# marvinquiet/SpaDOT

Hardware: AMD Instinct MI355X
Metric: training steps/sec + Sinkhorn iters/sec, 50k spots x 3k genes x 5 timepoints (higher is better)
Workload: dtype bf16; 1 GPU; cfg3: 5 time points x 10000 spots x 3000 genes, batch 512, k=30, 1200 inducing points; parallelism=1 GPU, n_sub=9980, E_sub=308893, m_inducing=236, params=16136032, hip_graphs=True, staged_graphs=True, bucketed_grad_exchange=False, units_in_schedule=80

## Files before the change

### include/spadot_model.h

```cpp
#ifndef SPADOT_MODEL_H
#define SPADOT_MODEL_H

#ifdef __cplusplus
extern "C" {
#endif

enum { SPADOT_DT_F32 = 0, SPADOT_DT_BF16 = 1, SPADOT_DT_F64 = 2 };
enum { SPADOT_KERNEL_GAUSSIAN = 0, SPADOT_KERNEL_CAUCHY = 1, SPADOT_KERNEL_QUADRATIC = 2 };

const char *spadot_model_version(void);

int spadot_gat_forward(const void *h, int dtype, const float *s_src, const float *s_dst,
                       const int *rowptr, const int *col, const float *bias, int n, int H, int C,
                       int concat, int act, void *out, float *alpha_out, void *stream);

int spadot_gat_backward_target(const void *g_out, const void *out, const void *h, int dtype,
                               const float *s_src, const float *s_dst, const float *alpha,
                               const int *rowptr, const int *col, int n, int H, int C, int concat,
                               int act, void *g_pre, float *dz, float *ds_dst, void *stream);

int spadot_gat_backward_source(const void *g_pre, int dtype, const float *alpha, const float *dz,
                               const int *rowptr_t, const int *col_t, const int *eid_t, int n, int H,
                               int C, void *dh, float *ds_src, const float *ds_dst, const float *att_src,
                               const float *att_dst, void *stream);
// ... 92 lines not shown
int spadot_kmeans_assign(const void *x, const void *centers, int n, int k, int d, int dtype, int *labels,
                         void *stream);

int spadot_sgemm_small(int mode, const float *A, int lda, const float *B, int ldb, float *C, int ldc, int M, int N, int K,
                       const float *bias, int batch, long long strideA, long long strideB, long long strideC, void *stream);

int spadot_enc_fused_supported(int b, int F1, int F2, int Q);
long long spadot_enc_fused_workspace(int b, int F1, int F2, int Q);
int spadot_enc_bn_map(const float *h1, const float *lin_bias, const float *gamma, const float *beta, float *running_mean,
                      float *running_var, long long *num_batches_tracked, int b, int F1, double momentum, double eps, double slope,
                      float *y1, float *save_mean, float *save_invstd, const float *W2, int F2, float *part, void *stream);
int spadot_enc_bn_fc(const float *part, int nparts, const float *lin_bias, const float *gamma, const float *beta, float *running_mean,
                     float *running_var, long long *num_batches_tracked, int b, int F2, double momentum, double eps, double slope,
                     float *h2, float *y2, float *save_mean, float *save_invstd, const float *Wfc, int Q, float *pz, void *stream);
int spadot_enc_sum_z(const float *pz, int nparts, const float *bias, int b, int Q, float *z, void *stream);
int spadot_svgp_pre2_partials(const float *pz, int nparts, const float *bias, const double *Kn, int b, int L, int m, float *z,
                              double *mu, double *var, double *w, double *muw, double *A, void *stream);

int spadot_recon_fb_supported(int b, int K, int G);
long long spadot_recon_fb_workspace(int b, int K, int G);
int spadot_recon_fb(const void *h_bf16, const void *W_bf16, const void *WT_bf16, int ldt, const float *bias, const float *y, int b, int K,
                    int G, double inv_scale, const float *grad_weight, void *g_bf16, float *workspace, double *loss_parts, float *dh,
                    void *stream);
int spadot_sum_parts(const double *part, int n, double scale, float *out, void *stream);

int spadot_stamp(unsigned long long *buf, int slot, void *stream);

int spadot_lloyd_step(const double *X, double *C, const int *xoff, const int *npts, int n_max, int R, const int *rgroup,
                      const int *Kr, int K_max, int D, const double *tol, double *part, int *done, double *inertia, int skip_done,
                      void *stream);
int spadot_kmeanspp_seed(const double *X, const int *xoff, const int *npts, int D, int P, const int *pset, const int *pK,
                         const int *pfirst, const int *puoff, const double *U, int K_max, int n_max, double *closest, int *idx,
                         double *centers, void *stream);

int spadot_knn(const double *x, int n, int d, int kk, int *out, void *stream);

int spadot_gat_mfma_supported(int dtype, int H, int C, int max_cols);

int spadot_gat_tail_supported(int dtype, int H, int K);
int spadot_gat_tail_wvec(const float *W, int ldw, const float *att_src, const float *att_dst, int H, int C, int K, float *part,
                         int slices, float *wv, void *whi, void *wlo, void *stream);
int spadot_gat_tail_logits(const void *x, int dtype, int ldx, const float *wv, const void *whi, const void *wlo, int n, int H, int K,
                           float *s, void *stream);
int spadot_gat_tail_aggregate(const void *x, int dtype, int ldx, const float *s, const int *rowptr, const int *col, int n_tgt, int H,
                              int K, void *A, float *alpha, void *stream);
int spadot_gat_tail_headmean(const void *O, int dtype, const float *bias, int n_tgt, int H, int C, void *out, void *stream);
// ... 37 lines not shown
int spadot_gemm_wgrad_bf16(const void *G, int ldg, const void *X, int ldx, float *dW, int ldw, int M, int N, int K,
                           int slices, float *workspace, const void *zero_row, void *stream);
long long spadot_gemm_wgrad_bf16_workspace_tiled(int M, int N, int K, int slices, int tile_k);
int spadot_gemm_wgrad_bf16_tiled(const void *G, int ldg, const void *X, int ldx, float *dW, int ldw, int M, int N, int K,
                                 int slices, int tile_k, float *workspace, const void *zero_row, void *stream);

int spadot_mlp_chain_supported(int n_layers, const int *dims);
int spadot_mlp_chain_workspace(int b, int n_layers, const int *dims, int *n_rows, int *width);
int spadot_mlp_chain_forward(const float *x, int b, int n_layers, const int *dims, const float *const *W,
                             const float *const *bias, const float *const *gamma, const float *const *beta, const double *eps,
                             const double *slope, float *const *a, float *const *y, float *const *mean, float *const *invstd,
                             void *stream);
int spadot_mlp_chain_forward_bf16(const float *x, int b, int n_layers, const int *dims, const float *const *W,
                                  const float *const *bias, const float *const *gamma, const float *const *beta,
                                  const double *eps, const double *slope, float *const *a, float *const *y, float *const *mean,
                                  float *const *invstd, void *y_last_bf16, void *stream);
int spadot_mlp_chain_backward(const float *dy, const float *x, int b, int n_layers, const int *dims, const float *const *W,
                              const float *const *gamma, const double *slope, float *const *a, float *const *y,
                              float *const *mean, float *const *invstd, float *dx, float *workspace, float *grads, void *stream);
int spadot_mlp_chain_backward_add(const float *dy, const float *x, int b, int n_layers, const int *dims, const float *const *W,
                                  const float *const *gamma, const double *slope, float *const *a, float *const *y,
                                  float *const *mean, float *const *invstd, float *dx, const float *dx_add, float *workspace,
                                  float *grads, void *stream);

int spadot_bias_sqerr_forward(const float *o, const float *bias, const float *y, int b, int G, double inv_scale, double *scratch,
                              float *out, void *stream);
int spadot_bias_sqerr_backward(const float *g1, const float *o, const float *bias, const float *y, int b, int G,
                               double inv_scale, void *g_bf16, float *dbias, void *stream);

int spadot_headfc_backward(const float *g, const void *h_bf16, const float *W, int b, int K, int N, void *dh_bf16,
                           float *workspace , float *grads ,
                           void *stream);

int spadot_cast_rows_multi(const float *const *src, void *const *dst, const int *rows, const int *K, const int *Kp, int n,
                           void *stream);

int spadot_grad_sumsq(const float *grad, long long count, double *scratch, float *sumsq, void *stream);
int spadot_clip_adamw_dev(float *param, const float *grad, float *exp_avg, float *exp_avg_sq, long long count, double lr,
                          double beta1, double beta2, double eps, double weight_decay, double max_norm, double *scratch,
                          float *sumsq, int *step_dev, unsigned *counter, const float *grad_scale_dev, void *stream);
typedef struct spadot_weight_image {
    long long offset;
    int rows, K, Kp, reserved;
    void *image;
} spadot_weight_image;
typedef struct spadot_weight_images {
// ... 79 lines not shown
```

### spadot_amd/_lib.py

```python
import ctypes
import os

_CSRC = os.path.join(os.path.dirname(os.path.abspath(__file__)), "csrc")
_CACHE = {}


class NativeLibraryMissing(RuntimeError):
    pass


def _load(name):
    if name in _CACHE:
        return _CACHE[name]
    import torch

    path = os.path.join(_CSRC, name)
    if not os.path.exists(path):
        raise NativeLibraryMissing(
            f"{path} is missing: build the HIP extension with `python -m spadot_amd.csrc.build` "
            "(needs hipcc; cross-compiles for gfx950 without a GPU). There is no CPU fallback.")
    lib = ctypes.CDLL(path)
    _CACHE[name] = lib
    return lib

# ... 148 lines not shown
        "spadot_gemm_tn_bf16": [vp, ci, vp, ci, vp, ci, ci, ci, ci, vp],
        "spadot_gemm_nn_bf16": [vp, ci, vp, ci, vp, ci, ci, ci, ci, vp],
        "spadot_enc_fused_supported": [ci, ci, ci, ci],
        "spadot_recon_fb_supported": [ci, ci, ci],
        "spadot_recon_fb": [vp, vp, vp, ci, vp, vp, ci, ci, ci, cd, vp, vp, vp, vp, vp, vp],
        "spadot_sum_parts": [vp, ci, cd, vp, vp],
        "spadot_enc_bn_map": [vp, vp, vp, vp, vp, vp, vp, ci, ci, cd, cd, cd, vp, vp, vp, vp, ci, vp, vp],
        "spadot_enc_bn_fc": [vp, ci, vp, vp, vp, vp, vp, vp, ci, ci, cd, cd, cd, vp, vp, vp, vp, vp, ci, vp, vp],
        "spadot_enc_sum_z": [vp, ci, vp, ci, ci, vp, vp],
        "spadot_svgp_pre2_partials": [vp, ci, vp, vp, ci, ci, ci, vp, vp, vp, vp, vp, vp, vp],
        "spadot_gemm_nn_bf16_masked": [vp, ci, vp, ci, vp, ci, ci, ci, ci, vp, ci, cd, vp],
        "spadot_gemm_tn_bf16_split": [vp, ci, vp, ci, vp, ci, ci, ci, ci, ci, ci, vp, vp],
        "spadot_gemm_wgrad_bf16": [vp, ci, vp, ci, vp, ci, ci, ci, ci, ci, vp, vp, vp],
        "spadot_gemm_wgrad_bf16_tiled": [vp, ci, vp, ci, vp, ci, ci, ci, ci, ci, ci, vp, vp, vp],
        "spadot_mlp_chain_supported": [ci, vp],
        "spadot_headfc_backward": [vp, vp, vp, ci, ci, ci, vp, vp, vp, vp],
        "spadot_bias_sqerr_forward": [vp, vp, vp, ci, ci, cd, vp, vp, vp],
        "spadot_bias_sqerr_backward": [vp, vp, vp, vp, ci, ci, cd, vp, vp, vp],
        "spadot_mlp_chain_workspace": [ci, ci, vp, vp, vp],
        "spadot_mlp_chain_forward": [vp, ci, ci, vp, vp, vp, vp, vp, vp, vp, vp, vp, vp, vp, vp],
        "spadot_mlp_chain_forward_bf16": [vp, ci, ci, vp, vp, vp, vp, vp, vp, vp, vp, vp, vp, vp, vp, vp],
        "spadot_mlp_chain_backward": [vp, vp, ci, ci, vp, vp, vp, vp, vp, vp, vp, vp, vp, vp, vp, vp],
        "spadot_mlp_chain_backward_add": [vp, vp, ci, ci, vp, vp, vp, vp, vp, vp, vp, vp, vp, vp, vp, vp, vp],
        "spadot_kernel_matrix": [vp, vp, ci, ci, ci, cd, ci, ci, vp, vp],
        "spadot_spd_inverse_logdet": [vp, ci, ci, vp, vp, vp],
        "spadot_rowdot_forward": [vp, vp, ci, ci, ci, ci, vp, vp],
        "spadot_rowdot_backward": [vp, vp, ci, ci, ci, ci, vp, vp],
        "spadot_elbo_forward": [vp, vp, vp, vp, vp, vp, vp, ci, ci, ci, vp, vp],
        "spadot_elbo_backward": [vp, vp, vp, vp, vp, vp, vp, vp, ci, ci, ci, vp, vp, vp, vp, vp, vp, vp],
        "spadot_bn_act_forward": [vp, ci, vp, vp, vp, vp, vp, vp, ci, ci, cd, cd, cd, vp, vp, vp, vp],
        "spadot_bn_act_backward": [vp, vp, vp, ci, vp, vp, vp, vp, ci, ci, cd, vp, vp, vp, vp],
        "spadot_ln_act_forward": [vp, vp, vp, ci, ci, cd, cd, vp, vp, vp, vp],
        "spadot_ln_act_backward": [vp, vp, vp, vp, vp, vp, ci, ci, cd, vp, vp, vp, vp],
        "spadot_svgp_post_forward": [vp] * 9 + [ci, ci, ci, cd, cd, cd] + [vp] * 7,
        "spadot_svgp_post_backward": [vp] * 13 + [ci, ci, ci, cd, cd] + [vp] * 8,
        "spadot_svgp_grad_tail": [vp] * 11 + [ci, ci, cd] + [vp] * 4,
        "spadot_svgp_q1t": [vp, vp, vp, vp, vp, ci, ci, ci, vp, vp],
        "spadot_svgp_post_pm_pv": [vp, vp, vp, ci, ci, cd, vp, vp, vp],
        "spadot_svgp_pre": [vp, ci, ci, vp, vp, vp, vp, vp],
        "spadot_svgp_pre2": [vp, vp, ci, ci, ci, vp, vp, vp, vp, vp, vp],
        "spadot_svgp_mid": [vp, vp, vp, vp, ci, ci, ci, vp, vp, vp, vp, vp, ci, vp],
        "spadot_spd_inverse_logdet2": [vp, ci, ci, ci, vp, vp, vp, vp, vp],
        "spadot_latent_head_forward": [vp, vp, vp, vp, ci, ci, ci, vp, vp, vp, vp, vp, vp],
        "spadot_latent_head_backward": [vp, vp, vp, vp, vp, vp, vp, ci, ci, ci, vp, vp, vp, vp],
        "spadot_cluster_losses_forward": [vp, vp, vp, vp, vp, vp, vp, ci, ci, ci, ci, ci, ci, ci, vp, vp, vp],
        "spadot_cluster_losses_backward": [vp, vp, vp, vp, vp, vp, vp, vp, ci, ci, ci, ci, ci, ci, ci, vp, vp],
# ... 64 lines not shown
```

### spadot_amd/csrc/mlp_chain.hip

```cpp
#include <hip/hip_runtime.h>
#include <cstdint>

#include "../../include/spadot_model.h"
#include "per_device.h"

namespace {

constexpr int MAXL = 4, MAXD = 256, WAVE = 64;
constexpr int RBF = 4;
constexpr int RBB = 8;
constexpr int LDW = MAXD + 4;

typedef float f32x4 __attribute__((ext_vector_type(4)));

struct Stage {
    const float *W, *bias, *gamma, *beta;
    float *a, *y, *mean, *invstd;
    int din, dout;
    float eps, slope;
    int ws_off;
};
struct Chain {
    Stage s[MAXL];
    int n;
// ... 58 lines not shown
            float ss = 0.f;
            for (int j = lane; j < dout; j += WAVE) { const float d = ar[j] - mean; ss += d * d; }
            const float invstd = rsqrtf(wave_sum(ss) / (float)dout + s.eps);
            for (int j = lane; j < dout; j += WAVE) {
                const float av = ar[j];
                const float v = (av - mean) * invstd * par[1][j] + par[2][j];
                const float yv = v > 0.f ? v : s.slope * v;
                ar[j] = yv;
                if (row < b) {
                    s.a[(size_t)row * dout + j] = av; s.y[(size_t)row * dout + j] = yv;
                    if (ch.ybf && l == ch.n - 1) ch.ybf[(size_t)row * dout + j] = (__bf16)yv;
                }
            }
            if (lane == 0 && row < b) { s.mean[row] = mean; s.invstd[row] = invstd; }
        }
        __syncthreads();
        cur ^= 1;
    }
}

constexpr int WST = 16384;
constexpr int LPR = 256 / RBB;
constexpr int LDS_BWD_FLOATS = 4 * RBB * LDW + 2 * RBB + MAXD + WST;
__global__ __launch_bounds__(256, 1) void k_mlp_chain_bwd(const float *__restrict__ dy_last, const float *__restrict__ x, int b,
                                                       Chain ch, float *__restrict__ dx_out, float *__restrict__ ws,
                                                       int ws_width, const float *__restrict__ dx_add) {
    extern __shared__ __attribute__((aligned(16))) float lds_dyn[];
    float (*gz)[LDW] = reinterpret_cast<float (*)[LDW]>(lds_dyn);
    float (*da)[LDW] = reinterpret_cast<float (*)[LDW]>(lds_dyn + RBB * LDW);
    float (*xs)[LDW] = reinterpret_cast<float (*)[LDW]>(lds_dyn + 2 * RBB * LDW);
    float (*xh)[LDW] = reinterpret_cast<float (*)[LDW]>(lds_dyn + 3 * RBB * LDW);
    float *rmean = lds_dyn + 4 * RBB * LDW, *rinv = rmean + RBB;
    float *gam = rinv + RBB;
    float *wst = gam + MAXD;
    const int t = threadIdx.x;
    const int r0 = blockIdx.x * RBB;
    float *wrow = ws + (size_t)blockIdx.x * ws_width;
    {
        const int d = ch.s[ch.n - 1].dout;
        float v[RBB * MAXD / 256];
#pragma unroll
        for (int u = 0; u < RBB * MAXD / 256; u++) {
            const int e = min(t + u * 256, RBB * d - 1), r = e / d, j = e - r * d;
            v[u] = dy_last[(size_t)min(r0 + r, b - 1) * d + j];
        }
#pragma unroll
        for (int u = 0; u < RBB * MAXD / 256; u++) {
            const int e = t + u * 256;
            if (!(e < RBB * d && r0 + e / d < b)) v[u] = 0.f;
        }
#pragma unroll
        for (int u = 0; u < RBB * MAXD / 256; u++) {
            const int e = t + u * 256, r = e / d, j = e - r * d;
            if (e < RBB * d) gz[r][j] = v[u];
        }
    }
    for (int l = ch.n - 1; l >= 0; l--) {
        const Stage &s = ch.s[l];
        const int din = s.din, dout = s.dout;
        const float *xin = l == 0 ? x : ch.s[l - 1].y;
        const int tk = din / 4;
        const int jc = min(dout, WST / din);
        const bool need_dx = l > 0 || dx_out != nullptr;
        {
            constexpr int NE = RBB * MAXD / 256, NW = WST / 4 / 256;
            float vx[NE], vy[NE], va[NE];
            f32x4 vw[NW];
#pragma unroll
            for (int u = 0; u < NE; u++) {
                const int e = min(t + u * 256, RBB * din - 1), r = e / din, k = e - r * din;
                vx[u] = xin[(size_t)min(r0 + r, b - 1) * din + k];
                const int e2 = min(t + u * 256, RBB * dout - 1), r2 = e2 / dout, j = e2 - r2 * dout;
                const size_t o2 = (size_t)min(r0 + r2, b - 1) * dout + j;
                vy[u] = s.y[o2];
                va[u] = s.a[o2];
            }
            {
                const f32x4 *src = reinterpret_cast<const f32x4 *>(s.W);
#pragma unroll
                for (int u = 0; u < NW; u++) vw[u] = src[min(t + u * 256, jc * tk - 1)];
            }
            const int rr = min(r0 + (t & (RBB - 1)), b - 1);
            const float mean_t = s.mean[rr], inv_t = s.invstd[rr], gam_t = s.gamma[min(t, dout - 1)];
#pragma unroll
            for (int u = 0; u < NE; u++) {
                const int e = t + u * 256;
                if (!(e < RBB * din && r0 + e / din < b)) vx[u] = 0.f;
                if (!(e < RBB * dout && r0 + e / dout < b)) { vy[u] = 0.f; va[u] = 0.f; }
            }
            if (t < RBB) {
                const bool live = r0 + t < b;
                rmean[t] = live ? mean_t : 0.f;
                rinv[t] = live ? inv_t : 0.f;
            }
            if (t < dout) gam[t] = gam_t;
            __syncthreads();
#pragma unroll
            for (int u = 0; u < NE; u++) {
                const int e = t + u * 256;
                if (e < RBB * din) { const int r = e / din; xs[r][e - r * din] = vx[u]; }
                if (e < RBB * dout) {
                    const int r = e / dout, j = e - r * dout;
                    const bool live = r0 + r < b;
                    gz[r][j] = live ? gz[r][j] * (vy[u] > 0.f ? 1.f : s.slope) : 0.f;
                    xh[r][j] = live ? (va[u] - rmean[r]) * rinv[r] : 0.f;
                }
// ... 94 lines not shown
                            const float4 w = *reinterpret_cast<const float4 *>(wst + (size_t)j * din + k0);
                            a4.x += d * w.x; a4.y += d * w.y; a4.z += d * w.z; a4.w += d * w.w;
                        }
                        acc[u] = a4;
                    }
                }
            }
#pragma unroll
            for (int u = 0; u < 4; u++) {
                const int e = it0 + u * 128;
                if (half == 1 && e < nitem) *reinterpret_cast<float4 *>(&xh[0][0] + 4 * e) = acc[u];
            }
            __syncthreads();
#pragma unroll
            for (int u = 0; u < 4; u++) {
                const int e = it0 + u * 128;
                if (half == 0 && e < nitem) {
                    const int r = e / tk, k0 = (e - r * tk) * 4;
                    const float4 o = *reinterpret_cast<const float4 *>(&xh[0][0] + 4 * e);
                    const float4 a4 = make_float4(acc[u].x + o.x, acc[u].y + o.y, acc[u].z + o.z, acc[u].w + o.w);
                    if (l > 0) *reinterpret_cast<float4 *>(&gz[r][k0]) = a4;
                    else if (r0 + r < b) {
                        float4 o4 = a4;
                        if (dx_add) {
                            const float4 e4 = *reinterpret_cast<const float4 *>(dx_add + (size_t)(r0 + r) * din + k0);
                            o4 = make_float4(a4.x + e4.x, a4.y + e4.y, a4.z + e4.z, a4.w + e4.w);
                        }
                        *reinterpret_cast<float4 *>(dx_out + (size_t)(r0 + r) * din + k0) = o4;
                    }
                }
            }
        }
        __syncthreads();
    }
}

__device__ __forceinline__ double block_sum_d(double x, double *sh) {
#pragma unroll
    for (int off = 32; off > 0; off >>= 1) x += __shfl_xor(x, off, WAVE);
    const int w = threadIdx.x >> 6, nw = (blockDim.x + 63) >> 6;
    __syncthreads();
    if ((threadIdx.x & 63) == 0) sh[w] = x;
    __syncthreads();
    double t = 0.0;
    for (int k = 0; k < nw; k++) t += sh[k];
    return t;
}

constexpr int SQ_ROWS = 1;
__global__ __launch_bounds__(256) void k_bias_sqerr_part(const float *__restrict__ o, const float *__restrict__ bias,
                                                         const float *__restrict__ y, int b, int G,
                                                         double *__restrict__ part) {
    __shared__ double sh[16];
    const size_t row = (size_t)blockIdx.x * G;
    double acc = 0.0;
    for (int c0 = threadIdx.x; c0 < G; c0 += 4 * 256) {
// ... 160 lines not shown
    *n_rows = (b + RBB - 1) / RBB;
    *width = w;
    return 0;
}

int spadot_mlp_chain_forward_bf16(const float *x, int b, int n_layers, const int *dims, const float *const *W,
                                  const float *const *bias, const float *const *gamma, const float *const *beta,
                                  const double *eps, const double *slope, float *const *a, float *const *y, float *const *mean,
                                  float *const *invstd, void *y_last_bf16, void *stream) {
    Chain ch;
    if (b <= 0 || !fill_chain(ch, n_layers, dims, W, bias, gamma, beta, eps, slope, a, y, mean, invstd)) return -22;
    ch.ybf = (__bf16 *)y_last_bf16;
    hipLaunchKernelGGL(k_mlp_chain_fwd, dim3((b + RBF - 1) / RBF), dim3(256), 0, (hipStream_t)stream, x, b, ch);
    return hipGetLastError() == hipSuccess ? 0 : -5;
}

int spadot_mlp_chain_forward(const float *x, int b, int n_layers, const int *dims, const float *const *W,
                             const float *const *bias, const float *const *gamma, const float *const *beta, const double *eps,
                             const double *slope, float *const *a, float *const *y, float *const *mean, float *const *invstd,
                             void *stream) {
    return spadot_mlp_chain_forward_bf16(x, b, n_layers, dims, W, bias, gamma, beta, eps, slope, a, y, mean, invstd, nullptr, stream);
}

int spadot_mlp_chain_backward_add(const float *dy, const float *x, int b, int n_layers, const int *dims, const float *const *W,
                                  const float *const *gamma, const double *slope, float *const *a, float *const *y,
                                  float *const *mean, float *const *invstd, float *dx, const float *dx_add, float *workspace,
                                  float *grads, void *stream) {
    Chain ch;
    if (b <= 0 || !fill_chain(ch, n_layers, dims, W, nullptr, gamma, nullptr, nullptr, slope, a, y, mean, invstd)) return -22;
    if (dx_add && !dx) return -22;
    int rows, width;
    if (spadot_mlp_chain_workspace(b, n_layers, dims, &rows, &width)) return -22;
    constexpr int LDS_BWD = LDS_BWD_FLOATS * (int)sizeof(float);
    static PerDeviceFlag attr_set;     
    if (!attr_set) {
        if (hipFuncSetAttribute((const void *)k_mlp_chain_bwd, hipFuncAttributeMaxDynamicSharedMemorySize, LDS_BWD) != hipSuccess) return -5;
        attr_set = true;
    }
    hipLaunchKernelGGL(k_mlp_chain_bwd, dim3(rows), dim3(256), LDS_BWD, (hipStream_t)stream, dy, x, b, ch, dx, workspace, width, dx_add);
    if (hipGetLastError() != hipSuccess) return -5;
    if (!grads) return 0;
    return spadot_colsum(workspace, rows, width, grads, stream);
}

int spadot_mlp_chain_backward(const float *dy, const float *x, int b, int n_layers, const int *dims, const float *const *W,
                              const float *const *gamma, const double *slope, float *const *a, float *const *y,
                              float *const *mean, float *const *invstd, float *dx, float *workspace, float *grads, void *stream) {
    return spadot_mlp_chain_backward_add(dy, x, b, n_layers, dims, W, gamma, slope, a, y, mean, invstd, dx, nullptr, workspace, grads,
                                         stream);
}

int spadot_bias_sqerr_forward(const float *o, const float *bias, const float *y, int b, int G, double inv_scale, double *scratch,
                              float *out, void *stream) {
    const int nb = (b + SQ_ROWS - 1) / SQ_ROWS;
    if (b <= 0 || G <= 0 || !scratch || nb > 4096) return -22;
    hipLaunchKernelGGL(k_bias_sqerr_part, dim3(nb), dim3(256), 0, (hipStream_t)stream, o, bias, y, b, G, scratch);
    hipLaunchKernelGGL(k_sum_parts, dim3(1), dim3(1024), 0, (hipStream_t)stream, scratch, nb, inv_scale, out);
    return hipGetLastError() == hipSuccess ? 0 : -5;
}

int spadot_bias_sqerr_backward(const float *g1, const float *o, const float *bias, const float *y, int b, int G,
                               double inv_scale, void *g_bf16, float *dbias, void *stream) {
    if (b <= 0 || G <= 0) return -22;
    hipLaunchKernelGGL(k_bias_sqerr_bwd, dim3((G + SB_COLS - 1) / SB_COLS), dim3(SB_COLS * SB_GY), 0, (hipStream_t)stream, g1, o,
                       bias, y, b, G, inv_scale, (__bf16 *)g_bf16, dbias);
// ... 16 lines not shown
```

### spadot_amd/csrc/recon_fb.hip

```cpp
#include <hip/hip_runtime.h>
#include <cmath>
#include <cstdint>

#include "../../include/spadot_model.h"

namespace {

constexpr int K = 256;
constexpr int BR = 64, BG = 128;
constexpr int NT = 256;
constexpr int DROW = 2 * BG + 16;
constexpr int LDS_D = BR * DROW;

typedef __bf16 bf8 __attribute__((ext_vector_type(8)));
typedef float f16v __attribute__((ext_vector_type(16)));

__device__ __forceinline__ unsigned short bf16_bits(float x) { return __builtin_bit_cast(unsigned short, (__bf16)x); }
__device__ __forceinline__ unsigned pack2(float lo, float hi) { return (unsigned)bf16_bits(lo) | ((unsigned)bf16_bits(hi) << 16); }

__global__ __launch_bounds__(NT, 1) void k_recon_fb(const __bf16 *__restrict__ hb, const __bf16 *__restrict__ W,
                                                    const __bf16 *__restrict__ WT, int ldt,
                                                    const float *__restrict__ bias, const float *__restrict__ y, int b, int G,
                                                    double inv_scale, const float *__restrict__ gw, __bf16 *__restrict__ gc,
                                                    float *__restrict__ dbp, double *__restrict__ lossp, float *__restrict__ dxp) {
// ... 124 lines not shown
        f32x4 v[8];
#pragma unroll
        for (int u = 0; u < 8; u++) v[u] = src[(long long)min(k + u, nblk - 1) * n4];
#pragma unroll
        for (int u = 0; u < 8; u++)
            if (k + u < nblk) acc += v[u];
    }
    reinterpret_cast<f32x4 *>(dh)[e] = acc;
}

}

extern "C" {

int spadot_recon_fb_supported(int b, int Kin, int G) {
    return b > 0 && b <= 4096 && Kin == K && G >= BG && G % 8 == 0;
}

long long spadot_recon_fb_workspace(int b, int Kin, int G) {
    if (!spadot_recon_fb_supported(b, Kin, G)) return -22;
    return (long long)((G + BG - 1) / BG) * b * K + (long long)((b + BR - 1) / BR) * G;
}

int spadot_recon_fb(const void *h_bf16, const void *W_bf16, const void *WT_bf16, int ldt, const float *bias, const float *y, int b, int Kin,
                    int G, double inv_scale, const float *grad_weight, void *g_bf16, float *workspace, double *loss_parts, float *dh,
                    void *stream) {
    if (!spadot_recon_fb_supported(b, Kin, G) || !h_bf16 || !W_bf16 || !WT_bf16 || !bias || !y || !grad_weight || !g_bf16 || !workspace ||
        !loss_parts || !dh || ldt < (G + BG - 1) / BG * BG || ldt % 8 || ((uintptr_t)WT_bf16 & 15))
        return -22;
    if (((uintptr_t)h_bf16 & 15) || ((uintptr_t)W_bf16 & 15) || ((uintptr_t)bias & 15) || ((uintptr_t)y & 15) || ((uintptr_t)g_bf16 & 15) ||
        ((uintptr_t)workspace & 15) || ((uintptr_t)dh & 15))
        return -22;
    const int GB = (G + BG - 1) / BG, RB = (b + BR - 1) / BR;
    float *dxp = workspace, *dbp = workspace + (size_t)GB * b * K;
    hipStream_t st = (hipStream_t)stream;
    hipLaunchKernelGGL(k_recon_fb, dim3(GB, RB), dim3(NT), 0, st, (const __bf16 *)h_bf16, (const __bf16 *)W_bf16, (const __bf16 *)WT_bf16, ldt,
                       bias, y, b, G,
                       inv_scale, grad_weight, (__bf16 *)g_bf16, dbp, loss_parts, dxp);
    const long long n4 = (long long)b * K / 4;
    hipLaunchKernelGGL(k_recon_fb_reduce, dim3((unsigned)((n4 + 255) / 256)), dim3(256), 0, st, (const float *)dxp, GB, n4, dh);
    return hipGetLastError() == hipSuccess ? 0 : -5;
}

}

namespace {
__global__ __launch_bounds__(256) void k_sum_parts_d(const double *__restrict__ part, int n, double scale, float *__restrict__ out) {
    __shared__ double sh[4];
    double acc = 0.0;
    for (int k = threadIdx.x; k < n; k += 256) acc += part[k];
#pragma unroll
    for (int off = 32; off > 0; off >>= 1) acc += __shfl_xor(acc, off, 64);
    if ((threadIdx.x & 63) == 0) sh[threadIdx.x >> 6] = acc;
    __syncthreads();
    if (threadIdx.x == 0) out[0] = (float)((((sh[0] + sh[1]) + sh[2]) + sh[3]) * scale);
}
}

extern "C" int spadot_sum_parts(const double *part, int n, double scale, float *out, void *stream) {
    if (!part || !out || n < 1) return -22;
    hipLaunchKernelGGL(k_sum_parts_d, dim3(1), dim3(256), 0, (hipStream_t)stream, part, n, scale, out);
    return hipGetLastError() == hipSuccess ? 0 : -5;
}
```

### spadot_amd/model/decoder.py

```python
import torch
import torch.nn as nn
import torch.nn.functional as F

from ..ops import (grad_bias, linear_bias, ln_act, mlp_chain, mlp_chain_ok, recon_fb_ok, recon_sqerr, recon_sqerr_fb, recon_sqerr_ok,
                   sqerr_sum, weight_image)


def _hidden_stage(fan_in, fan_out):
    dense = nn.Linear(fan_in, fan_out)
    nn.init.xavier_uniform_(dense.weight)
    return dense, nn.LayerNorm(fan_out), nn.LeakyReLU()


class Decoder(nn.Module):
    def __init__(self, input_dim, z_dim, decoder_layers, compute_dtype=torch.float32):
        super().__init__()
        self.compute_dtype = compute_dtype
        widths = [z_dim, *decoder_layers]
        stages = []
        for fan_in, fan_out in zip(widths[:-1], widths[1:]):
            stages.extend(_hidden_stage(fan_in, fan_out))
        stages.append(nn.Linear(widths[-1], input_dim))
        self.decoder_net = nn.Sequential(*stages)

    def forward(self, latent_sample):
        h, last, _ = self._hidden(latent_sample)
        return linear_bias(h, last.weight, last.bias, self.compute_dtype)

    def recon_loss(self, latent_sample, y, inv_scale, dz_extra=None, grad_weight=None):
        bf = self.compute_dtype == torch.bfloat16
        nocast = bf
        h, last, hb = self._hidden(latent_sample, bf16_out=nocast, dx_add=dz_extra)
        if bf and grad_weight is not None:
            wim = self._output_image(last.weight)
            wimT = self._output_image_T(wim) if wim is not None else None
            if recon_fb_ok(h, last.weight, last.bias, y, hb, wim, wimT, grad_weight):
                return recon_sqerr_fb(h, last.weight, last.bias, y, inv_scale, hb, wim, wimT, grad_weight)
        if bf and recon_sqerr_ok(h, last.weight, last.bias, y):
            return recon_sqerr(h, last.weight, last.bias, y, inv_scale, hb, self._output_image(last.weight) if nocast else None)
        return sqerr_sum(y, linear_bias(h, last.weight, last.bias, self.compute_dtype), inv_scale)

    def _output_image(self, W):
        opt = getattr(self, "_image_optimizer", None)
        if opt is None or not self.training or not W.is_cuda:
            return None
        if not opt.owns(W):
            object.__setattr__(self, "_image_optimizer", None)
            return None
        im = weight_image(W, W.shape[1], torch.bfloat16, self, tag="_wout")
        if not opt.maintain_image(W, im):
            return None
        opt.sync_images()
        return im

    def _output_image_T(self, wim, refresh=None):
        G, K = wim.shape
        Gp = (G + 127) // 128 * 128
        t = getattr(self, "_wout_T", None)
        if t is None or t.shape != (K, Gp) or t.device != wim.device:
            t = torch.zeros((K, Gp), dtype=torch.bfloat16, device=wim.device)
# ... 31 lines not shown
```

### spadot_amd/ops.py

```python
import ctypes

import torch

from ._lib import model_lib

DT_F32, DT_BF16, DT_F64 = 0, 1, 2
_DT = {torch.float32: DT_F32, torch.bfloat16: DT_BF16, torch.float64: DT_F64}
KERNEL_KINDS = {"Gaussian": 0, "Cauchy": 1, "Quadratic": 2}


def _p(t):
    return ctypes.c_void_p(t.data_ptr()) if t is not None else None


def _stream():
    return ctypes.c_void_p(torch.cuda.current_stream().cuda_stream)


def _need_cuda(*ts):
    for t in ts:
        if t is not None and not t.is_cuda:
            raise RuntimeError("spadot_amd ops run on the MI355X only (got a CPU tensor); there is no CPU path")


# ... 886 lines not shown
MLP_CHAIN = [True]


def _ptr_array(tensors):
    return (ctypes.c_void_p * len(tensors))(*(t_.data_ptr() for t_ in tensors))


def _contiguous_grad_block(params):
    gs_ = [p.grad for p in params]
    if any(g is None or g.dtype != torch.float32 or not g.is_contiguous() for g in gs_):
        return None
    st0, off = gs_[0].untyped_storage(), gs_[0].storage_offset()
    pos = off
    for g in gs_:
        if g.untyped_storage().data_ptr() != st0.data_ptr() or g.storage_offset() != pos:
            return None
        pos += g.numel()
    return torch.empty(0, dtype=torch.float32, device=gs_[0].device).set_(st0, off, (pos - off,))


CHAIN_BF16_OUT = [False]
CHAIN_DX_ADD = [None]
_LAST_CHAIN_BF16 = []


class _MLPChain(torch.autograd.Function):

    @staticmethod
    def forward(ctx, x, eps, slope, *params):
        n = len(params) // 4
        Ws, bs, gs, betas = params[0::4], params[1::4], params[2::4], params[3::4]
        b = x.shape[0]
        dims = [x.shape[1]] + [W.shape[0] for W in Ws]
        dev = x.device
        a = [torch.empty((b, d), dtype=torch.float32, device=dev) for d in dims[1:]]
        y = [torch.empty((b, d), dtype=torch.float32, device=dev) for d in dims[1:]]
        stats = torch.empty((2 * n, b), dtype=torch.float32, device=dev)
        mean, inv = [stats[2 * l] for l in range(n)], [stats[2 * l + 1] for l in range(n)]
        cd = (ctypes.c_int * (n + 1))(*dims)
        ce = (ctypes.c_double * n)(*[float(e) for e in eps])
        cs = (ctypes.c_double * n)(*[float(v) for v in slope])
        ybf = torch.empty((b, dims[-1]), dtype=torch.bfloat16, device=dev) if CHAIN_BF16_OUT[0] else None
        _check(model_lib().spadot_mlp_chain_forward_bf16(_p(x), b, n, cd, _ptr_array(Ws), _ptr_array(bs), _ptr_array(gs),
                                                         _ptr_array(betas), ce, cs, _ptr_array(a), _ptr_array(y), _ptr_array(mean),
                                                         _ptr_array(inv), None if ybf is None else _p(ybf), _stream()),
               "spadot_mlp_chain_forward_bf16")
# ... 6 lines not shown
        return y[-1]

    @staticmethod
    def backward(ctx, dy):
        n, dims = ctx.n, ctx.dims
        sv = ctx.saved_tensors
        x, stats = sv[0], sv[1]
        Ws, gs, a, y = sv[2:2 + n], sv[2 + n:2 + 2 * n], sv[2 + 2 * n:2 + 3 * n], sv[2 + 3 * n:2 + 4 * n]
        b = x.shape[0]
        dev = x.device
        cd = (ctypes.c_int * (n + 1))(*dims)
        rows, width = ctypes.c_int(0), ctypes.c_int(0)
        lib = model_lib()
        _check(lib.spadot_mlp_chain_workspace(b, n, cd, ctypes.byref(rows), ctypes.byref(width)), "spadot_mlp_chain_workspace")
        ws = torch.empty((rows.value, width.value), dtype=torch.float32, device=dev)
        direct = ctx.flat_out is not None and _DIRECT_GRAD[0] and ctx.flat_out.numel() == width.value
        grads = ctx.flat_out if direct else torch.empty(width.value, dtype=torch.float32, device=dev)
        dx = torch.empty_like(x) if ctx.needs_input_grad[0] else None
        mean, inv = [stats[2 * l] for l in range(n)], [stats[2 * l + 1] for l in range(n)]
        cs = (ctypes.c_double * n)(*ctx.slope)
        late = direct and _deferring()
        add = ctx.dx_add
        assert add is None or (dx is not None and add.shape == x.shape and add.dtype == torch.float32 and add.is_contiguous())
        _check(lib.spadot_mlp_chain_backward_add(_p(dy.contiguous().float()), _p(x), b, n, cd, _ptr_array(Ws), _ptr_array(gs), cs,
                                                 _ptr_array(a), _ptr_array(y), _ptr_array(mean), _ptr_array(inv),
                                                 None if dx is None else _p(dx), None if add is None else _p(add), _p(ws),
                                                 None if late else _p(grads), _stream()),
               "spadot_mlp_chain_backward_add")
        if late:
            DEFERRED[0].append(lambda ws=ws, grads=grads: _check(
                lib.spadot_colsum(_p(ws), ws.shape[0], ws.shape[1], _p(grads), _stream()), "spadot_colsum"))
        out = []
        off = 0
        for l in range(n):
            din, dout = dims[l], dims[l + 1]
            out += [grads[off:off + dout * din].view(dout, din), grads[off + dout * din:off + dout * din + dout],
                    grads[off + dout * din + dout:off + dout * din + 2 * dout],
                    grads[off + dout * din + 2 * dout:off + dout * din + 3 * dout]]
            off += dout * din + 3 * dout
        return (dx, None, None, *out)


def mlp_chain_ok(x, stages):
    if not (MLP_CHAIN[0] and x.is_cuda and x.dtype == torch.float32 and x.dim() == 2 and 1 <= len(stages) <= 4):
        return False
    dims = [x.shape[1]] + [lin.out_features for lin, _, _ in stages]
    if any(lin.in_features != d for (lin, _, _), d in zip(stages, dims[:-1])):
        return False
    ts = [t_ for lin, ln, _ in stages for t_ in (lin.weight, lin.bias, ln.weight, ln.bias)]
    if any(t_ is None or t_.dtype != torch.float32 or not t_.is_contiguous() or t_.data_ptr() % 16 for t_ in ts):
        return False
# ... 457 lines not shown
    def backward(ctx, g):
        hc, Wc, o, bias, y = ctx.saved_tensors
        b, G = y.shape
        g1 = g.reshape(1).contiguous().float()
        gc = torch.empty((b, G), dtype=torch.bfloat16, device=y.device)
        direct = _DIRECT_GRAD[0]
        db = ctx.bgrad if (direct and ctx.bgrad is not None) else torch.empty(G, dtype=torch.float32, device=y.device)
        _check(model_lib().spadot_bias_sqerr_backward(_p(g1), _p(o), _p(bias), _p(y), b, G, ctx.inv_scale, _p(gc), _p(db),
                                                      _stream()), "spadot_bias_sqerr_backward")
        dh = torch.mm(gc, Wc, out_dtype=torch.float32) if ctx.needs_input_grad[0] else None
        if direct and ctx.wgrad is not None and _deferring():
            DEFERRED[0].append(lambda gc=gc, hc=hc, out=ctx.wgrad: torch.mm(gc.t(), hc, out_dtype=torch.float32, out=out))
            dW = ctx.wgrad
        elif direct and ctx.wgrad is not None:
            dW = torch.mm(gc.t(), hc, out_dtype=torch.float32, out=ctx.wgrad)
        else:
            dW = torch.mm(gc.t(), hc, out_dtype=torch.float32)
        return dh, dW, db, None, None, None, None


class _ReconFB(torch.autograd.Function):

    @staticmethod
    def forward(ctx, h, W, bias, y, inv_scale, hc, Wc, WcT, gw):
        lib = model_lib()
        b, K = h.shape
        G = W.shape[0]
        dev = h.device
        nfl = int(lib.spadot_recon_fb_workspace(b, K, G))
        GB, RB = (G + 127) // 128, (b + 63) // 64
        ws = torch.empty(nfl, dtype=torch.float32, device=dev)
        lossp = torch.empty(GB * RB, dtype=torch.float64, device=dev)
        gc = torch.empty((b, G), dtype=torch.bfloat16, device=dev)
        dh = torch.empty((b, K), dtype=torch.float32, device=dev)
        _check(lib.spadot_recon_fb(_p(hc), _p(Wc), _p(WcT), WcT.shape[1], _p(bias), _p(y), b, K, G, float(inv_scale), _p(gw), _p(gc), _p(ws),
                                   _p(lossp), _p(dh), _stream()), "spadot_recon_fb")
        out = torch.empty(1, dtype=torch.float32, device=dev)

        def value(lossp=lossp, out=out):
            _check(lib.spadot_sum_parts(_p(lossp), GB * RB, float(inv_scale), _p(out), _stream()), "spadot_sum_parts")

        if DEFERRED[0] is not None:
            DEFERRED[0].append(value)
        else:
            value()
        ctx.save_for_backward(hc, gc, dh)
        ctx.dbp = ws[GB * b * K:].view(RB, G)
        ctx.seed = gw.data_ptr()
        ok = lambda g_, p_: g_ if (g_ is not None and g_.dtype == torch.float32 and g_.is_contiguous() and g_.shape == p_.shape) else None
        ctx.wgrad, ctx.bgrad = ok(W.grad, W), ok(bias.grad, bias)
        return out[0]

    @staticmethod
    def backward(ctx, g):
        if g is None or g.data_ptr() != ctx.seed:
            raise RuntimeError("recon_sqerr_fb: backward seeded with something other than the weight its gradient was formed for "
                               "(the forward launch already holds d loss / d h for THAT seed)")
        hc, gc, dh = ctx.saved_tensors
        lib = model_lib()
        dbp = ctx.dbp
        direct = _DIRECT_GRAD[0]
        db = ctx.bgrad if (direct and ctx.bgrad is not None) else torch.empty(dbp.shape[1], dtype=torch.float32, device=dh.device)
        dW = ctx.wgrad if (direct and ctx.wgrad is not None) else torch.empty((gc.shape[1], hc.shape[1]), dtype=torch.float32, device=dh.device)

        def rest(dbp=dbp, db=db, dW=dW, gc=gc, hc=hc):
            _check(lib.spadot_colsum(_p(dbp), dbp.shape[0], dbp.shape[1], _p(db), _stream()), "spadot_colsum")
            torch.mm(gc.t(), hc, out_dtype=torch.float32, out=dW)

        if direct and ctx.wgrad is not None and ctx.bgrad is not None and _deferring():
            DEFERRED[0].append(rest)
        else:
            with torch.no_grad():
                rest()
        return dh, dW, db, None, None, None, None, None, None


def recon_fb_ok(h, W, bias, y, hc, Wc, WcT, gw):
    ok = lambda t_, like: (t_ is not None and t_.dtype == torch.bfloat16 and t_.is_contiguous() and t_.shape == like.shape)
    okT = (WcT is not None and WcT.dtype == torch.bfloat16 and WcT.is_contiguous() and WcT.dim() == 2 and WcT.shape[0] == W.shape[1]
           and WcT.shape[1] >= (W.shape[0] + 127) // 128 * 128 and WcT.shape[1] % 8 == 0 and WcT.data_ptr() % 16 == 0)
    return bool(okT and gw is not None and gw.is_cuda and gw.dtype == torch.float32 and h.is_cuda and h.dtype == torch.float32 and h.dim() == 2
                and y.dtype == torch.float32 and y.is_contiguous() and y.shape == (h.shape[0], W.shape[0]) and bias is not None
                and bias.dtype == torch.float32 and bias.is_contiguous() and bias.data_ptr() % 16 == 0 and y.data_ptr() % 16 == 0
                and ok(hc, h) and ok(Wc, W) and model_lib().spadot_recon_fb_supported(h.shape[0], h.shape[1], W.shape[0]))


def recon_sqerr_fb(h, W, bias, y, inv_scale, h_bf16, W_image, W_image_T, grad_weight):
    return _ReconFB.apply(h, W, bias, y, inv_scale, h_bf16, W_image, W_image_T, grad_weight)


def recon_sqerr_ok(h, W, bias, y):
    return bool(h.is_cuda and h.dtype == torch.float32 and y.dtype == torch.float32 and h.dim() == 2
                and y.dim() == 2 and h.shape[1] % 4 == 0 and W.shape[1] % 4 == 0 and y.shape == (h.shape[0], W.shape[0])
                and h.shape[0] <= 4096
                and bias is not None)


def recon_sqerr(h, W, bias, y, inv_scale, h_bf16=None, W_image=None):
    ok = lambda t_, like: (t_ is not None and t_.dtype == torch.bfloat16 and t_.is_contiguous() and t_.shape == like.shape)
    return _LinearSqErr.apply(h.contiguous(), W, bias, y.contiguous(), inv_scale, h_bf16 if ok(h_bf16, h) else None,
                              W_image if ok(W_image, W) else None)


def kmeans_assign(x, centers):
    _need_cuda(x, centers)
    x = x.contiguous()
    centers = centers.contiguous().to(x.dtype)
    labels = torch.empty(x.shape[0], dtype=torch.int32, device=x.device)
    _check(model_lib().spadot_kmeans_assign(_p(x), _p(centers), x.shape[0], centers.shape[0], x.shape[1],
                                            _DT[x.dtype], _p(labels), _stream()), "spadot_kmeans_assign")
    return labels
# ... 390 lines not shown
```

Before: 668.0 training steps/s.

## Fuse recon dh partial reduction into MLP chain backward and prefetch stage loads

The reconstruction kernel no longer launches its own reduction of per-column-block dh partials. Those partials are handed to the MLP chain backward kernel, which sums them on load, removing one kernel launch and a full dh write and read. The chain backward also prefetches the next stage's inputs, weights and the dx_add tile into registers while the current stage computes. In exchange, register pressure rises, and passing the partials through a side dictionary keyed by pointer is fragile.

Result: no change. 666.3 training steps/s (-0.3%).

```diff
diff --git a/include/spadot_model.h b/include/spadot_model.h
--- a/include/spadot_model.h
+++ b/include/spadot_model.h
@@ -138,6 +138,7 @@
 int spadot_recon_fb(const void *h_bf16, const void *W_bf16, const void *WT_bf16, int ldt, const float *bias, const float *y, int b, int K,
                     int G, double inv_scale, const float *grad_weight, void *g_bf16, float *workspace, double *loss_parts, float *dh,
                     void *stream);
+int spadot_recon_fb_reduce(const float *workspace, int b, int K, int G, float *dh, void *stream);
 int spadot_sum_parts(const double *part, int n, double scale, float *out, void *stream);
 
 int spadot_stamp(unsigned long long *buf, int slot, void *stream);
@@ -221,6 +222,10 @@
                                   const float *const *gamma, const double *slope, float *const *a, float *const *y,
                                   float *const *mean, float *const *invstd, float *dx, const float *dx_add, float *workspace,
                                   float *grads, void *stream);
+int spadot_mlp_chain_backward_parts(const float *dy_parts, int nparts, long long part_stride, const float *x, int b, int n_layers,
+                                    const int *dims, const float *const *W, const float *const *gamma, const double *slope,
+                                    float *const *a, float *const *y, float *const *mean, float *const *invstd, float *dx,
+                                    const float *dx_add, float *workspace, float *grads, void *stream);
 
 int spadot_bias_sqerr_forward(const float *o, const float *bias, const float *y, int b, int G, double inv_scale, double *scratch,
                               float *out, void *stream);
diff --git a/spadot_amd/_lib.py b/spadot_amd/_lib.py
--- a/spadot_amd/_lib.py
+++ b/spadot_amd/_lib.py
@@ -194,6 +194,8 @@
         "spadot_mlp_chain_forward_bf16": [vp, ci, ci, vp, vp, vp, vp, vp, vp, vp, vp, vp, vp, vp, vp, vp],
         "spadot_mlp_chain_backward": [vp, vp, ci, ci, vp, vp, vp, vp, vp, vp, vp, vp, vp, vp, vp, vp],
         "spadot_mlp_chain_backward_add": [vp, vp, ci, ci, vp, vp, vp, vp, vp, vp, vp, vp, vp, vp, vp, vp, vp],
+        "spadot_mlp_chain_backward_parts": [vp, ci, ll, vp, ci, ci, vp, vp, vp, vp, vp, vp, vp, vp, vp, vp, vp, vp, vp],
+        "spadot_recon_fb_reduce": [vp, ci, ci, ci, vp, vp],
         "spadot_kernel_matrix": [vp, vp, ci, ci, ci, cd, ci, ci, vp, vp],
         "spadot_spd_inverse_logdet": [vp, ci, ci, vp, vp, vp],
         "spadot_rowdot_forward": [vp, vp, ci, ci, ci, ci, vp, vp],
diff --git a/spadot_amd/csrc/mlp_chain.hip b/spadot_amd/csrc/mlp_chain.hip
--- a/spadot_amd/csrc/mlp_chain.hip
+++ b/spadot_amd/csrc/mlp_chain.hip
@@ -104,7 +104,43 @@
 constexpr int WST = 16384;
 constexpr int LPR = 256 / RBB;
 constexpr int LDS_BWD_FLOATS = 4 * RBB * LDW + 2 * RBB + MAXD + WST;
-__global__ __launch_bounds__(256, 1) void k_mlp_chain_bwd(const float *__restrict__ dy_last, const float *__restrict__ x, int b,
+constexpr int NE = RBB * MAXD / 256;
+constexpr int NW = WST / 4 / 256;
+constexpr int DYC = 12;
+
+struct StageRegs {
+    float vx[NE], vy[NE], va[NE];
+    f32x4 vw[NW];
+    float mean_t, inv_t, gam_t;
+};
+
+__device__ __forceinline__ void load_stage(StageRegs &R, const Chain &ch, const float *__restrict__ x, int l, int live, int t, int r0,
+                                           int b) {
+    const Stage &s = ch.s[l];
+    const int din = s.din, dout = s.dout;
+    const float *xin = l == 0 ? x : ch.s[max(l - 1, 0)].y;
+    const int tk = din / 4;
+    const int jc = min(dout, WST / din);
+#pragma unroll
+    for (int u = 0; u < NE; u++) {
+        const int e = min(t + u * 256, RBB * din - 1) * live, r = e / din, k = e - r * din;
+        R.vx[u] = xin[(size_t)min(r0 + r, b - 1) * din + k];
+        const int e2 = min(t + u * 256, RBB * dout - 1) * live, r2 = e2 / dout, j = e2 - r2 * dout;
+        const size_t o2 = (size_t)min(r0 + r2, b - 1) * dout + j;
+        R.vy[u] = s.y[o2];
+        R.va[u] = s.a[o2];
+    }
+    {
+        const f32x4 *src = reinterpret_cast<const f32x4 *>(s.W);
+#pragma unroll
+        for (int u = 0; u < NW; u++) R.vw[u] = src[min(t + u * 256, jc * tk - 1) * live];
+    }
+    const int rr = min(r0 + (t & (RBB - 1)), b - 1);
+    R.mean_t = s.mean[rr]; R.inv_t = s.invstd[rr]; R.gam_t = s.gamma[min(t, dout - 1)];
+}
+
+__global__ __launch_bounds__(256, 1) void k_mlp_chain_bwd(const float *__restrict__ dy_parts, int nparts, long long pstride,
+                                                       const float *__restrict__ x, int b,
                                                        Chain ch, float *__restrict__ dx_out, float *__restrict__ ws,
                                                        int ws_width, const float *__restrict__ dx_add) {
     extern __shared__ __attribute__((aligned(16))) float lds_dyn[];
@@ -118,21 +154,59 @@
     const int t = threadIdx.x;
     const int r0 = blockIdx.x * RBB;
     float *wrow = ws + (size_t)blockIdx.x * ws_width;
+    StageRegs cur, nxt;
+    f32x4 ea[4];
     {
         const int d = ch.s[ch.n - 1].dout;
-        float v[RBB * MAXD / 256];
-#pragma unroll
-        for (int u = 0; u < RBB * MAXD / 256; u++) {
+        size_t off[NE];
+#pragma unroll
+        for (int u = 0; u < NE; u++) {
             const int e = min(t + u * 256, RBB * d - 1), r = e / d, j = e - r * d;
-            v[u] = dy_last[(size_t)min(r0 + r, b - 1) * d + j];
-        }
-#pragma unroll
-        for (int u = 0; u < RBB * MAXD / 256; u++) {
+            off[u] = (size_t)min(r0 + r, b - 1) * d + j;
+        }
+        float pv[DYC][NE];
+#pragma unroll
+        for (int q = 0; q < DYC; q++) {
+            const float *pp = dy_parts + (size_t)min(q, nparts - 1) * (size_t)pstride;
+#pragma unroll
+            for (int u = 0; u < NE; u++) pv[q][u] = pp[off[u]];
+        }
+        load_stage(cur, ch, x, ch.n - 1, 1, t, r0, b);
+        {
+            const int din0 = ch.s[0].din, tk0 = din0 / 4;
+            const float *addp = dx_add ? dx_add : x;
+#pragma unroll
+            for (int u = 0; u < 4; u++) {
+                const int e = min((t & 127) + u * 128, RBB * tk0 - 1), r = e / tk0, k0 = (e - r * tk0) * 4;
+                ea[u] = *reinterpret_cast<const f32x4 *>(addp + (size_t)min(r0 + r, b - 1) * din0 + k0);
+            }
+        }
+        float v[NE];
+#pragma unroll
+        for (int u = 0; u < NE; u++) v[u] = nparts > 1 ? 0.f : -0.f;
+#pragma unroll
+        for (int q = 0; q < DYC; q++)
+#pragma unroll
+            for (int u = 0; u < NE; u++) v[u] += q < nparts ? pv[q][u] : -0.f;
+        for (int k = DYC; k < nparts; k += DYC) {
+#pragma unroll
+            for (int q = 0; q < DYC; q++) {
+                const float *pp = dy_parts + (size_t)min(k + q, nparts - 1) * (size_t)pstride;
+#pragma unroll
+                for (int u = 0; u < NE; u++) pv[q][u] = pp[off[u]];
+            }
+#pragma unroll
+            for (int q = 0; q < DYC; q++)
+#pragma unroll
+                for (int u = 0; u < NE; u++) v[u] += k + q < nparts ? pv[q][u] : -0.f;
+        }
+#pragma unroll
+        for (int u = 0; u < NE; u++) {
             const int e = t + u * 256;
             if (!(e < RBB * d && r0 + e / d < b)) v[u] = 0.f;
         }
 #pragma unroll
-        for (int u = 0; u < RBB * MAXD / 256; u++) {
+        for (int u = 0; u < NE; u++) {
             const int e = t + u * 256, r = e / d, j = e - r * d;
             if (e < RBB * d) gz[r][j] = v[u];
         }
@@ -140,30 +214,14 @@
     for (int l = ch.n - 1; l >= 0; l--) {
         const Stage &s = ch.s[l];
         const int din = s.din, dout = s.dout;
-        const float *xin = l == 0 ? x : ch.s[l - 1].y;
         const int tk = din / 4;
         const int jc = min(dout, WST / din);
         const bool need_dx = l > 0 || dx_out != nullptr;
+        load_stage(nxt, ch, x, max(l - 1, 0), l > 0 ? 1 : 0, t, r0, b);
         {
-            constexpr int NE = RBB * MAXD / 256, NW = WST / 4 / 256;
-            float vx[NE], vy[NE], va[NE];
-            f32x4 vw[NW];
-#pragma unroll
-            for (int u = 0; u < NE; u++) {
-                const int e = min(t + u * 256, RBB * din - 1), r = e / din, k = e - r * din;
-                vx[u] = xin[(size_t)min(r0 + r, b - 1) * din + k];
-                const int e2 = min(t + u * 256, RBB * dout - 1), r2 = e2 / dout, j = e2 - r2 * dout;
-                const size_t o2 = (size_t)min(r0 + r2, b - 1) * dout + j;
-                vy[u] = s.y[o2];
-                va[u] = s.a[o2];
-            }
-            {
-                const f32x4 *src = reinterpret_cast<const f32x4 *>(s.W);
-#pragma unroll
-                for (int u = 0; u < NW; u++) vw[u] = src[min(t + u * 256, jc * tk - 1)];
-            }
-            const int rr = min(r0 + (t & (RBB - 1)), b - 1);
-            const float mean_t = s.mean[rr], inv_t = s.invstd[rr], gam_t = s.gamma[min(t, dout - 1)];
+            float (&vx)[NE] = cur.vx, (&vy)[NE] = cur.vy, (&va)[NE] = cur.va;
+            f32x4 (&vw)[NW] = cur.vw;
+            const float mean_t = cur.mean_t, inv_t = cur.inv_t, gam_t = cur.gam_t;
 #pragma unroll
             for (int u = 0; u < NE; u++) {
                 const int e = t + u * 256;
@@ -304,16 +362,15 @@
                     if (l > 0) *reinterpret_cast<float4 *>(&gz[r][k0]) = a4;
                     else if (r0 + r < b) {
                         float4 o4 = a4;
-                        if (dx_add) {
-                            const float4 e4 = *reinterpret_cast<const float4 *>(dx_add + (size_t)(r0 + r) * din + k0);
-                            o4 = make_float4(a4.x + e4.x, a4.y + e4.y, a4.z + e4.z, a4.w + e4.w);
-                        }
+                        if (dx_add)
+                            o4 = make_float4(a4.x + ea[u].x, a4.y + ea[u].y, a4.z + ea[u].z, a4.w + ea[u].w);
                         *reinterpret_cast<float4 *>(dx_out + (size_t)(r0 + r) * din + k0) = o4;
                     }
                 }
             }
         }
         __syncthreads();
+        cur = nxt;
     }
 }
 
@@ -520,13 +577,14 @@
     return spadot_mlp_chain_forward_bf16(x, b, n_layers, dims, W, bias, gamma, beta, eps, slope, a, y, mean, invstd, nullptr, stream);
 }
 
-int spadot_mlp_chain_backward_add(const float *dy, const float *x, int b, int n_layers, const int *dims, const float *const *W,
-                                  const float *const *gamma, const double *slope, float *const *a, float *const *y,
-                                  float *const *mean, float *const *invstd, float *dx, const float *dx_add, float *workspace,
-                                  float *grads, void *stream) {
+int spadot_mlp_chain_backward_parts(const float *dy_parts, int nparts, long long part_stride, const float *x, int b, int n_layers,
+                                    const int *dims, const float *const *W, const float *const *gamma, const double *slope,
+                                    float *const *a, float *const *y, float *const *mean, float *const *invstd, float *dx,
+                                    const float *dx_add, float *workspace, float *grads, void *stream) {
     Chain ch;
-    if (b <= 0 || !fill_chain(ch, n_layers, dims, W, nullptr, gamma, nullptr, nullptr, slope, a, y, mean, invstd)) return -22;
+    if (b <= 0 || !dy_parts || nparts < 1 || !fill_chain(ch, n_layers, dims, W, nullptr, gamma, nullptr, nullptr, slope, a, y, mean, invstd)) return -22;
     if (dx_add && !dx) return -22;
+    if (nparts > 1 && part_stride < (long long)b * dims[n_layers]) return -22;
     int rows, width;
     if (spadot_mlp_chain_workspace(b, n_layers, dims, &rows, &width)) return -22;
     constexpr int LDS_BWD = LDS_BWD_FLOATS * (int)sizeof(float);
@@ -535,10 +593,19 @@
         if (hipFuncSetAttribute((const void *)k_mlp_chain_bwd, hipFuncAttributeMaxDynamicSharedMemorySize, LDS_BWD) != hipSuccess) return -5;
         attr_set = true;
     }
-    hipLaunchKernelGGL(k_mlp_chain_bwd, dim3(rows), dim3(256), LDS_BWD, (hipStream_t)stream, dy, x, b, ch, dx, workspace, width, dx_add);
+    hipLaunchKernelGGL(k_mlp_chain_bwd, dim3(rows), dim3(256), LDS_BWD, (hipStream_t)stream, dy_parts, nparts, part_stride,
+                       x, b, ch, dx, workspace, width, dx_add);
     if (hipGetLastError() != hipSuccess) return -5;
     if (!grads) return 0;
     return spadot_colsum(workspace, rows, width, grads, stream);
+}
+
+int spadot_mlp_chain_backward_add(const float *dy, const float *x, int b, int n_layers, const int *dims, const float *const *W,
+                                  const float *const *gamma, const double *slope, float *const *a, float *const *y,
+                                  float *const *mean, float *const *invstd, float *dx, const float *dx_add, float *workspace,
+                                  float *grads, void *stream) {
+    return spadot_mlp_chain_backward_parts(dy, 1, 0, x, b, n_layers, dims, W, gamma, slope, a, y, mean, invstd, dx, dx_add, workspace,
+                                           grads, stream);
 }
 
 int spadot_mlp_chain_backward(const float *dy, const float *x, int b, int n_layers, const int *dims, const float *const *W,
diff --git a/spadot_amd/csrc/recon_fb.hip b/spadot_amd/csrc/recon_fb.hip
--- a/spadot_amd/csrc/recon_fb.hip
+++ b/spadot_amd/csrc/recon_fb.hip
@@ -170,11 +170,19 @@
     return (long long)((G + BG - 1) / BG) * b * K + (long long)((b + BR - 1) / BR) * G;
 }
 
+int spadot_recon_fb_reduce(const float *workspace, int b, int Kin, int G, float *dh, void *stream) {
+    if (!spadot_recon_fb_supported(b, Kin, G) || !workspace || !dh || ((uintptr_t)workspace & 15) || ((uintptr_t)dh & 15)) return -22;
+    const long long n4 = (long long)b * K / 4;
+    hipLaunchKernelGGL(k_recon_fb_reduce, dim3((unsigned)((n4 + 255) / 256)), dim3(256), 0, (hipStream_t)stream, workspace,
+                       (G + BG - 1) / BG, n4, dh);
+    return hipGetLastError() == hipSuccess ? 0 : -5;
+}
+
 int spadot_recon_fb(const void *h_bf16, const void *W_bf16, const void *WT_bf16, int ldt, const float *bias, const float *y, int b, int Kin,
                     int G, double inv_scale, const float *grad_weight, void *g_bf16, float *workspace, double *loss_parts, float *dh,
                     void *stream) {
     if (!spadot_recon_fb_supported(b, Kin, G) || !h_bf16 || !W_bf16 || !WT_bf16 || !bias || !y || !grad_weight || !g_bf16 || !workspace ||
-        !loss_parts || !dh || ldt < (G + BG - 1) / BG * BG || ldt % 8 || ((uintptr_t)WT_bf16 & 15))
+        !loss_parts || ldt < (G + BG - 1) / BG * BG || ldt % 8 || ((uintptr_t)WT_bf16 & 15))
         return -22;
     if (((uintptr_t)h_bf16 & 15) || ((uintptr_t)W_bf16 & 15) || ((uintptr_t)bias & 15) || ((uintptr_t)y & 15) || ((uintptr_t)g_bf16 & 15) ||
         ((uintptr_t)workspace & 15) || ((uintptr_t)dh & 15))
@@ -185,9 +193,8 @@
     hipLaunchKernelGGL(k_recon_fb, dim3(GB, RB), dim3(NT), 0, st, (const __bf16 *)h_bf16, (const __bf16 *)W_bf16, (const __bf16 *)WT_bf16, ldt,
                        bias, y, b, G,
                        inv_scale, grad_weight, (__bf16 *)g_bf16, dbp, loss_parts, dxp);
-    const long long n4 = (long long)b * K / 4;
-    hipLaunchKernelGGL(k_recon_fb_reduce, dim3((unsigned)((n4 + 255) / 256)), dim3(256), 0, st, (const float *)dxp, GB, n4, dh);
-    return hipGetLastError() == hipSuccess ? 0 : -5;
+    if (hipGetLastError() != hipSuccess) return -5;
+    return dh ? spadot_recon_fb_reduce(workspace, b, Kin, G, dh, stream) : 0;
 }
 
 }
diff --git a/spadot_amd/model/decoder.py b/spadot_amd/model/decoder.py
--- a/spadot_amd/model/decoder.py
+++ b/spadot_amd/model/decoder.py
@@ -35,7 +35,7 @@
             wim = self._output_image(last.weight)
             wimT = self._output_image_T(wim) if wim is not None else None
             if recon_fb_ok(h, last.weight, last.bias, y, hb, wim, wimT, grad_weight):
-                return recon_sqerr_fb(h, last.weight, last.bias, y, inv_scale, hb, wim, wimT, grad_weight)
+                return recon_sqerr_fb(h, last.weight, last.bias, y, inv_scale, hb, wim, wimT, grad_weight, h_from_chain=hb is not None)
         if bf and recon_sqerr_ok(h, last.weight, last.bias, y):
             return recon_sqerr(h, last.weight, last.bias, y, inv_scale, hb, self._output_image(last.weight) if nocast else None)
         return sqerr_sum(y, linear_bias(h, last.weight, last.bias, self.compute_dtype), inv_scale)
diff --git a/spadot_amd/ops.py b/spadot_amd/ops.py
--- a/spadot_amd/ops.py
+++ b/spadot_amd/ops.py
@@ -932,6 +932,8 @@
 CHAIN_BF16_OUT = [False]
 CHAIN_DX_ADD = [None]
 _LAST_CHAIN_BF16 = []
+CHAIN_DY_PARTS = [True]
+_DY_PARTS = {}
 
 
 class _MLPChain(torch.autograd.Function):
@@ -984,11 +986,17 @@
         late = direct and _deferring()
         add = ctx.dx_add
         assert add is None or (dx is not None and add.shape == x.shape and add.dtype == torch.float32 and add.is_contiguous())
-        _check(lib.spadot_mlp_chain_backward_add(_p(dy.contiguous().float()), _p(x), b, n, cd, _ptr_array(Ws), _ptr_array(gs), cs,
-                                                 _ptr_array(a), _ptr_array(y), _ptr_array(mean), _ptr_array(inv),
-                                                 None if dx is None else _p(dx), None if add is None else _p(add), _p(ws),
-                                                 None if late else _p(grads), _stream()),
-               "spadot_mlp_chain_backward_add")
+        parts = _DY_PARTS.pop(dy.data_ptr(), None) if _DY_PARTS else None
+        if parts is not None:
+            assert dy.dtype == torch.float32 and dy.is_contiguous() and parts.shape[1:] == dy.shape, "a partial gradient's handle was changed on its way"
+            src, nparts, pstride = parts, parts.shape[0], parts.stride(0)
+        else:
+            src, nparts, pstride = dy.contiguous().float(), 1, 0
+        _check(lib.spadot_mlp_chain_backward_parts(_p(src), nparts, pstride, _p(x), b, n, cd, _ptr_array(Ws), _ptr_array(gs), cs,
+                                                   _ptr_array(a), _ptr_array(y), _ptr_array(mean), _ptr_array(inv),
+                                                   None if dx is None else _p(dx), None if add is None else _p(add), _p(ws),
+                                                   None if late else _p(grads), _stream()),
+               "spadot_mlp_chain_backward_parts")
         if late:
             DEFERRED[0].append(lambda ws=ws, grads=grads: _check(
                 lib.spadot_colsum(_p(ws), ws.shape[0], ws.shape[1], _p(grads), _stream()), "spadot_colsum"))
@@ -1492,7 +1500,7 @@
 class _ReconFB(torch.autograd.Function):
 
     @staticmethod
-    def forward(ctx, h, W, bias, y, inv_scale, hc, Wc, WcT, gw):
+    def forward(ctx, h, W, bias, y, inv_scale, hc, Wc, WcT, gw, dh_parts):
         lib = model_lib()
         b, K = h.shape
         G = W.shape[0]
@@ -1502,9 +1510,10 @@
         ws = torch.empty(nfl, dtype=torch.float32, device=dev)
         lossp = torch.empty(GB * RB, dtype=torch.float64, device=dev)
         gc = torch.empty((b, G), dtype=torch.bfloat16, device=dev)
-        dh = torch.empty((b, K), dtype=torch.float32, device=dev)
+        ctx.parts = ws[:GB * b * K].view(GB, b, K) if dh_parts else None
+        dh = ctx.parts[0] if dh_parts else torch.empty((b, K), dtype=torch.float32, device=dev)
         _check(lib.spadot_recon_fb(_p(hc), _p(Wc), _p(WcT), WcT.shape[1], _p(bias), _p(y), b, K, G, float(inv_scale), _p(gw), _p(gc), _p(ws),
-                                   _p(lossp), _p(dh), _stream()), "spadot_recon_fb")
+                                   _p(lossp), None if dh_parts else _p(dh), _stream()), "spadot_recon_fb")
         out = torch.empty(1, dtype=torch.float32, device=dev)
 
         def value(lossp=lossp, out=out):
@@ -1529,6 +1538,10 @@
         hc, gc, dh = ctx.saved_tensors
         lib = model_lib()
         dbp = ctx.dbp
+        if ctx.parts is not None:
+            if _DY_PARTS:
+                raise RuntimeError("recon_sqerr_fb: an earlier partial gradient was never taken by the chain it was promised to")
+            _DY_PARTS[dh.data_ptr()] = ctx.parts
         direct = _DIRECT_GRAD[0]
         db = ctx.bgrad if (direct and ctx.bgrad is not None) else torch.empty(dbp.shape[1], dtype=torch.float32, device=dh.device)
         dW = ctx.wgrad if (direct and ctx.wgrad is not None) else torch.empty((gc.shape[1], hc.shape[1]), dtype=torch.float32, device=dh.device)
@@ -1542,7 +1555,7 @@
         else:
             with torch.no_grad():
                 rest()
-        return dh, dW, db, None, None, None, None, None, None
+        return dh, dW, db, None, None, None, None, None, None, None
 
 
 def recon_fb_ok(h, W, bias, y, hc, Wc, WcT, gw):
@@ -1555,8 +1568,9 @@
                 and ok(hc, h) and ok(Wc, W) and model_lib().spadot_recon_fb_supported(h.shape[0], h.shape[1], W.shape[0]))
 
 
-def recon_sqerr_fb(h, W, bias, y, inv_scale, h_bf16, W_image, W_image_T, grad_weight):
-    return _ReconFB.apply(h, W, bias, y, inv_scale, h_bf16, W_image, W_image_T, grad_weight)
+def recon_sqerr_fb(h, W, bias, y, inv_scale, h_bf16, W_image, W_image_T, grad_weight, h_from_chain=False):
+    parts = bool(h_from_chain and CHAIN_DY_PARTS[0] and type(h.grad_fn).__name__ == "_MLPChainBackward")
+    return _ReconFB.apply(h, W, bias, y, inv_scale, h_bf16, W_image, W_image_T, grad_weight, parts)
 
 
 def recon_sqerr_ok(h, W, bias, y):
```
